# tqch/ddpm-torch

Measured on AMD Instinct MI355X. Metric: training imgs/s/GPU + 1000-step DDPM samples/s, CIFAR-10 UNet @1/2/4/8 MI355X, higher is better.
Workload: dtype bf16; 1 GPU; configs/cifar10.json UNet (35.7M params), full Trainer.step, B=128 per GPU, 32x32, T=1000, dropout 0.1, Adam+clip+EMA; global_batch=128, rccl_ranks=1, parallelism=dp1

## Files before the change

ddpm-torch_amd/csrc/attention.hip:

```cpp
#include "common.h"
#include <string.h>

namespace {

constexpr int RB = 128;
constexpr int NT = 512;

struct Opnd {
    __amdgpu_buffer_rsrc_t rsrc;
    long long ld;
};

__device__ __forceinline__ Opnd make_opnd(const bf16_t* base, long long ld, int L, int C) {
    Opnd o;
    const UniformAddr u = uniform_addr(base);
    o.rsrc = buffer_rsrc_at(u, (unsigned)(((long long)(L - 1) * ld + C) * 2));
    o.ld = ld;
    return o;
}
__device__ __forceinline__ u32x4 ldv(const Opnd& o, unsigned off) {
    return __builtin_bit_cast(u32x4, __builtin_amdgcn_raw_buffer_load_b128(o.rsrc, off, 0, 0));
}
__device__ __forceinline__ bf16x8 as_frag(const u32x4& v) { return __builtin_bit_cast(bf16x8, v); }

struct AttnArgs {
    const bf16_t *q, *k, *v;  long long qkv_ld;
    const bf16_t *o, *d_o;    long long o_ld, do_ld;
    bf16_t *out;              long long out_ld;
    bf16_t *dq, *dk, *dv;     long long dqkv_ld;
    float *lse, *dvec;
    int B, L, C, Lpad;
    float scale;
};

__device__ __forceinline__ int tile_addr(int row, int col, int pitch_b, int km) {
    return row * pitch_b + ((((col >> 3) ^ (row & km))) << 4) + (col & 7) * 2;
}

template <int NJ>
struct P1 {
    f32x16 acc[2][NJ];
    __device__ __forceinline__ void zero() {
#pragma unroll
        for (int i = 0; i < 2; ++i)
#pragma unroll
            for (int j = 0; j < NJ; ++j) acc[i][j] = (f32x16)(0.f);
    }
};

__device__ __forceinline__ void wait_vm_rt(int n) {
    switch (n) {
    case 0: asm volatile("s_waitcnt vmcnt(0)" ::: "memory"); break;
    case 1: asm volatile("s_waitcnt vmcnt(1)" ::: "memory"); break;
    case 2: asm volatile("s_waitcnt vmcnt(2)" ::: "memory"); break;
    case 3: asm volatile("s_waitcnt vmcnt(3)" ::: "memory"); break;
    case 4: asm volatile("s_waitcnt vmcnt(4)" ::: "memory"); break;
    case 5: asm volatile("s_waitcnt vmcnt(5)" ::: "memory"); break;
    case 6: asm volatile("s_waitcnt vmcnt(6)" ::: "memory"); break;
    case 7: asm volatile("s_waitcnt vmcnt(7)" ::: "memory"); break;
    default: asm volatile("s_waitcnt vmcnt(8)" ::: "memory"); break;
    }
}

#ifdef ATTN_TIMING
__device__ unsigned long long* g_attn_timing = nullptr;
#define ATTN_STAMP(slot) do { if (g_attn_timing && threadIdx.x == 0) g_attn_timing[(blockIdx.y * gridDim.x + blockIdx.x) * 8 + (slot)] = wall_clock64(); } while (0)
#else
#define ATTN_STAMP(slot)
#endif

constexpr int P1_RING = 3, P2_RING = 5;
constexpr int P2_SLOT = 2 * NT * 16;
__device__ __host__ __forceinline__ int p1_slot_bytes(int Lpad) { return RB * 128 + ((Lpad + 63) / 64) * 8192; }
__device__ __host__ __forceinline__ int p2_rows(int C) { return C > 256 ? 16 : (C > 128 ? 32 : 64); }

template <int NJ, bool PIPE = true>
__device__ __forceinline__ void product_nt(P1<NJ>& t, const Opnd& X, int r0, const Opnd& Y, int Lpad, int C, char* lds, int tid) {
    const int lane = tid & 63, wr = (tid >> 8) & 1, wc = (tid >> 6) & 3;
    const int wave = __builtin_amdgcn_readfirstlane(tid >> 6);
    const int nyi = (Lpad + 63) / 64;
    const int xs_bytes = RB * 128, slot_bytes = p1_slot_bytes(Lpad), per = 2 + nyi;
    const unsigned lds0 = lds_addr(lds);
    const int nchunks = (C + 63) / 64;
    unsigned xo[2], yo[4]; int xc[2], yc[4];
#pragma unroll
    for (int i = 0; i < 2; ++i) {
        const int v = tid + NT * i, row = v >> 3;
        xc[i] = ((v & 7) ^ ((row >> 1) & 7)) * 8;
        xo[i] = (unsigned)(((long long)(r0 + row) * X.ld + xc[i]) * 2);
    }
#pragma unroll
    for (int i = 0; i < 4; ++i) {
        const int v = tid + NT * i, row = v >> 3;
        yc[i] = ((v & 7) ^ ((row >> 1) & 7)) * 8;
        yo[i] = row < Lpad ? (unsigned)(((long long)row * Y.ld + yc[i]) * 2) : BUF_OOB;
    }
    auto issue = [&](int ch) {
        char* slot = lds + (ch % P1_RING) * slot_bytes;
        const int c0 = ch * 64;
#pragma unroll
        for (int i = 0; i < 2; ++i) {
            unsigned o = c0 + xc[i] < C ? xo[i] + (unsigned)(c0 * 2) : BUF_OOB;
            asm volatile("" : "+v"(o));
            LDS_DMA16(X.rsrc, slot + (i * NT + wave * 64) * 16, o, 0);
        }
#pragma unroll
        for (int i = 0; i < 4; ++i) {
            if (i < nyi) {
                unsigned o = (yo[i] != BUF_OOB && c0 + yc[i] < C) ? yo[i] + (unsigned)(c0 * 2) : BUF_OOB;
                asm volatile("" : "+v"(o));
                LDS_DMA16(Y.rsrc, slot + xs_bytes + (i * NT + wave * 64) * 16, o, 0);
            }
        }
    };
    issue(0);
    if (nchunks > 1) issue(1);
    const int sw = (lane >> 5) ^ ((lane >> 1) & 7);
    const unsigned arow = (unsigned)((wr * 64 + (lane & 31)) * 128), brow = (unsigned)(xs_bytes + (wc * 32 + (lane & 31)) * 128);
    bool jok[NJ];
#pragma unroll
    for (int j = 0; j < NJ; ++j) jok[j] = (wc + 4 * j) * 32 < Lpad;
#ifdef ATTN_TIMING
    unsigned long long tq[5] = {0, 0, 0, 0, 0};
#define P1_T(k) do { if (ch == 1) tq[k] = clock64(); } while (0)
#else
#define P1_T(k)
#endif
    for (int ch = 0; ch < nchunks; ++ch) {
        P1_T(0);
        wait_vm_rt(ch + 1 < nchunks ? per : 0);
        P1_T(1);
        __builtin_amdgcn_s_barrier();
        P1_T(2);
        if (ch + 2 < nchunks) issue(ch + 2);
        P1_T(3);
        const unsigned cur = lds0 + (unsigned)((ch % P1_RING) * slot_bytes);
        constexpr int NS = PIPE ? 2 : 1;
        u32x4 fa[NS][2], fb[NS][NJ];
        auto rd = [&](int kc, int set) {
            const unsigned ko = (unsigned)(((2 * kc) ^ sw) << 4);
#pragma unroll
            for (int i = 0; i < 2; ++i) fa[set][i] = lds_rd16(cur + arow + (unsigned)(i * 32 * 128) + ko);
#pragma unroll
            for (int j = 0; j < NJ; ++j) fb[set][j] = lds_rd16(cur + (jok[j] ? brow + (unsigned)(j * 128 * 128) : (unsigned)xs_bytes) + ko);
        };
        rd(0, 0);
#pragma unroll
        for (int kc = 0; kc < 4; ++kc) {
            constexpr int cs = NS == 2 ? 1 : 0;
            if (NS == 1) { if (kc > 0) rd(kc, 0); lds_wait_n<0>(); }
            else if (kc < 3) { rd(kc + 1, (kc + 1) & 1); lds_wait_n<2 + NJ>(); } else lds_wait_n<0>();
#pragma unroll
            for (int i = 0; i < 2; ++i)
#pragma unroll
                for (int j = 0; j < NJ; ++j)
                    if (jok[j]) t.acc[i][j] = __builtin_amdgcn_mfma_f32_32x32x16_bf16(as_frag(fa[kc & cs][i]), as_frag(fb[kc & cs][j]), t.acc[i][j], 0, 0, 0);
            __builtin_amdgcn_sched_barrier(0);
        }
        P1_T(4);
    }
#ifdef ATTN_TIMING
    if (g_attn_timing && threadIdx.x == 0 && tq[4])
        g_attn_timing[(blockIdx.y * gridDim.x + blockIdx.x) * 8 + 7] = ((tq[1] - tq[0]) & 0xffff) | (((tq[2] - tq[1]) & 0xffff) << 16) | (((tq[3] - tq[2]) & 0xffff) << 32) | (((tq[4] - tq[3]) & 0xffff) << 48);
#endif
#undef P1_T
    __syncthreads();
}

template <int NJ2>
__device__ __forceinline__ void product_nn(f32x16 (&z)[2][NJ2], const char* tile, int pitch_b, int km, const Opnd& Y, int L, int Lpad, int C,
                                           char* ring, int tid) {
    const int lane = tid & 63, wr = (tid >> 8) & 1, wc = (tid >> 6) & 3;
    const int wave = __builtin_amdgcn_readfirstlane(tid >> 6);
    const int KR = p2_rows(C);
    const int row_b = C * 2, cpr = C >> 3;
    const int nvec = KR * cpr;
    const int skey = C % 128 == 0 ? 2 : 0;
#pragma unroll
    for (int i = 0; i < 2; ++i)
#pragma unroll
        for (int j = 0; j < NJ2; ++j) z[i][j] = (f32x16)(0.f);
    const int nchunks = (Lpad + KR - 1) / KR;
    int vkr[2]; unsigned vo[2];
#pragma unroll
    for (int i = 0; i < 2; ++i) {
        const int v = tid + NT * i;
        const int kr = v / cpr, pc = v - kr * cpr;
        const int lc = skey ? (pc ^ ((kr & 3) << 2)) : pc;
        vkr[i] = v < nvec ? kr : (1 << 20);
        vo[i] = (unsigned)(((long long)kr * Y.ld + lc * 8) * 2);
    }
    const unsigned kstep = (unsigned)((long long)KR * Y.ld * 2);
    auto issue = [&](int ch) {
        char* slot = ring + (ch % P2_RING) * P2_SLOT;
#pragma unroll
        for (int i = 0; i < 2; ++i) {
            unsigned o = ch * KR + vkr[i] < L ? vo[i] + (unsigned)ch * kstep : BUF_OOB;
            asm volatile("" : "+v"(o));
            LDS_DMA16(Y.rsrc, slot + (i * NT + wave * 64) * 16, o, 0);
        }
    };
    for (int c = 0; c < P2_RING - 1 && c < nchunks; ++c) issue(c);
    const int i16 = lane & 15;
    const unsigned tile0 = lds_addr(tile), ring0 = lds_addr(ring);
    bool jok[NJ2];
#pragma unroll
    for (int j = 0; j < NJ2; ++j) jok[j] = (wc + 4 * j) * 32 < C;
    for (int ch = 0; ch < nchunks; ++ch) {
        const int ahead = min(ch + P2_RING - 2, nchunks - 1) - ch;
        wait_vm_rt(2 * ahead);
        __builtin_amdgcn_s_barrier();
        if (ch + P2_RING - 1 < nchunks) issue(ch + P2_RING - 1);
        const unsigned cur = ring0 + (unsigned)((ch % P2_RING) * P2_SLOT);
        constexpr int NS = NJ2 <= 2 ? 2 : 1;
        u32x4 fa[NS][2]; uint2 fb[NS][NJ2][2];
        const int nks = min(KR / 16, (Lpad - ch * KR + 15) / 16);
        auto rd = [&](int ks, int set) {
            const int kg = ch * KR + ks * 16;
#pragma unroll
            for (int i = 0; i < 2; ++i) {
                const int row = wr * 64 + i * 32 + (lane & 31);
                fa[set][i] = lds_rd16(tile0 + (unsigned)(row * pitch_b + ((((kg >> 3) + (lane >> 5)) ^ (row & km)) << 4)));
            }
#pragma unroll
            for (int j = 0; j < NJ2; ++j) {
                const int ct = jok[j] ? wc + 4 * j : wc;
                const int mcol = ct * 32 + ((lane >> 4) & 1) * 16 + (i16 & 3) * 4;
                const int krow = ks * 16 + (lane >> 5) * 8 + (i16 >> 2);
                const int pch = skey ? ((mcol >> 3) ^ ((krow & 3) << 2)) : (mcol >> 3);
                const unsigned p = cur + (unsigned)(krow * row_b + pch * 16 + (mcol & 7) * 2);
                fb[set][j][0] = lds_rd_tr(p); fb[set][j][1] = lds_rd_tr(p + (unsigned)(4 * row_b));
            }
        };
        rd(0, 0);
        for (int ks = 0; ks < nks; ks += 2) {
#pragma unroll
            for (int h = 0; h < 2; ++h) {
                if (ks + h >= nks) break;
                constexpr int cs = NS == 2 ? 1 : 0;
                const int cur_set = h & cs;
                if (NS == 1) { if (ks + h > 0) rd(ks + h, 0); lds_wait_n<0>(); }
                else if (ks + h + 1 < nks) { rd(ks + h + 1, (h + 1) & 1); lds_wait_n<2 + 2 * NJ2>(); } else lds_wait_n<0>();
#pragma unroll
                for (int j = 0; j < NJ2; ++j) {
                    if (!jok[j]) continue;
                    u32x4 b4; b4.x = fb[cur_set][j][0].x; b4.y = fb[cur_set][j][0].y; b4.z = fb[cur_set][j][1].x; b4.w = fb[cur_set][j][1].y;
#pragma unroll
                    for (int i = 0; i < 2; ++i) z[i][j] = __builtin_amdgcn_mfma_f32_32x32x16_bf16(as_frag(fa[cur_set][i]), as_frag(b4), z[i][j], 0, 0, 0);
                }
                __builtin_amdgcn_sched_barrier(0);
            }
        }
    }
    __syncthreads();
}

template <int CNT, int OFF, typename Op>
__device__ __forceinline__ float half_reduce(const float (&v)[CNT], int lane, Op&& op) {
    if constexpr (CNT == 1) return v[0];
    else {
        const bool bit = (lane & OFF) != 0;
        float o[CNT / 2];
#pragma unroll
        for (int k = 0; k < CNT / 2; ++k) {
            const float send = bit ? v[k] : v[k + CNT / 2], keep = bit ? v[k + CNT / 2] : v[k];
            o[k] = op(keep, __shfl_xor(send, OFF, 64));
        }
        return half_reduce<CNT / 2, OFF / 2>(o, lane, op);
    }
}

__device__ __forceinline__ int acc_row(int r, int lane) { return (r & 3) + 8 * (r >> 2) + 4 * (lane >> 5); }

template <int NJ, typename F>
__device__ __forceinline__ void write_tile(const P1<NJ>& t, char* tile, int pitch_b, int km, int Lpad, int tid, F&& f) {
    const int lane = tid & 63, wave = tid >> 6, wr = wave >> 2, wc = wave & 3;
#pragma unroll
    for (int i = 0; i < 2; ++i)
#pragma unroll
        for (int j = 0; j < NJ; ++j) {
            const int ct = wc + 4 * j;
            if (ct * 32 >= Lpad) continue;
#pragma unroll
            for (int r = 0; r < 16; ++r) {
                const int row = wr * 64 + i * 32 + acc_row(r, lane), col = ct * 32 + (lane & 31);
                *reinterpret_cast<bf16_t*>(tile + tile_addr(row, col, pitch_b, km)) = f2bf(f(t.acc[i][j][r], i, j, r, row, col));
            }
        }
}

template <int NJ2>
__device__ __forceinline__ void store_rows(const f32x16 (&z)[2][NJ2], bf16_t* out, long long ld, int r0, int L, int C, int tid) {
    const int lane = tid & 63, wave = tid >> 6, wr = wave >> 2, wc = wave & 3;
#pragma unroll
    for (int i = 0; i < 2; ++i)
#pragma unroll
        for (int j = 0; j < NJ2; ++j) {
            const int ct = wc + 4 * j;
            if (ct * 32 >= C) continue;
#pragma unroll
            for (int r = 0; r < 16; ++r) {
                const int row = r0 + wr * 64 + i * 32 + acc_row(r, lane);
                if (row < L) out[(long long)row * ld + ct * 32 + (lane & 31)] = f2bf(z[i][j][r]);
            }
        }
}

__device__ __forceinline__ void attn_block(int B, int& b, int& r0) {
    const int gx = gridDim.x;
    if (gx > 1 && (B & 7) == 0) {
        const int L = blockIdx.y * gx + blockIdx.x, k = L >> 3;
        r0 = (k % gx) * RB;
        b = (k / gx) * 8 + (L & 7);
    } else { b = blockIdx.y; r0 = blockIdx.x * RB; }
}

struct Lds {
    char* tile; char* stage; float* red;
    int pitch_b, km;
};
__device__ __forceinline__ Lds carve(char* smem, int Lpad) {
    Lds l;
    l.pitch_b = Lpad * 2;
    const int nch = Lpad >> 3;
    int span = 4;
    while (span < 16 && nch % (span * 2) == 0) span *= 2;
    l.km = span - 1;
    l.tile = smem;
    l.stage = smem + RB * l.pitch_b;
    l.red = nullptr;
    return l;
}

template <int NJ1, int NJ2>
__global__ __launch_bounds__(NT, 2)
void attn_fwd_lse_kernel(AttnArgs a) {
    extern __shared__ __attribute__((aligned(16))) char smem[];
    const int tid = threadIdx.x, lane = tid & 63, wave = tid >> 6, wr = wave >> 2, wc = wave & 3;
    int b, r0;
    attn_block(a.B, b, r0);
    Lds l = carve(smem, a.Lpad);
    const Opnd Q = make_opnd(a.q + (long long)b * a.L * a.qkv_ld, a.qkv_ld, a.L, a.C);
    const Opnd K = make_opnd(a.k + (long long)b * a.L * a.qkv_ld, a.qkv_ld, a.L, a.C);
    const Opnd V = make_opnd(a.v + (long long)b * a.L * a.qkv_ld, a.qkv_ld, a.L, a.C);
    ATTN_STAMP(0);
    P1<NJ1> s;
    s.zero();
    product_nt<NJ1, (NJ2 <= 2)>(s, Q, r0, K, a.Lpad, a.C, smem, tid);
    ATTN_STAMP(1);
    float* red = reinterpret_cast<float*>(l.stage);
    const int kk = lane & 31, myrow = wr * 64 + (kk >> 4) * 32 + acc_row(kk & 15, lane);
    float vals[32];
#pragma unroll
    for (int i = 0; i < 2; ++i)
#pragma unroll
        for (int r = 0; r < 16; ++r) {
            float m = -3.0e38f;
#pragma unroll
            for (int j = 0; j < NJ1; ++j) {
                const int col = (wc + 4 * j) * 32 + (lane & 31);
                const float v = col < a.L ? s.acc[i][j][r] * a.scale : -3.0e38f;
                s.acc[i][j][r] = v;
                m = fmaxf(m, v);
            }
            vals[i * 16 + r] = m;
        }
    red[wc * RB + myrow] = half_reduce<32, 16>(vals, lane, [](float x, float y) { return fmaxf(x, y); });
    __syncthreads();
#pragma unroll
    for (int i = 0; i < 2; ++i)
#pragma unroll
        for (int r = 0; r < 16; ++r) {
            const int row = wr * 64 + i * 32 + acc_row(r, lane);
            const float m = fmaxf(fmaxf(red[row], red[RB + row]), fmaxf(red[2 * RB + row], red[3 * RB + row]));
            float sum = 0.f;
#pragma unroll
            for (int j = 0; j < NJ1; ++j) {
                const int col = (wc + 4 * j) * 32 + (lane & 31);
                const float e = col < a.L ? __expf(s.acc[i][j][r] - m) : 0.f;
                s.acc[i][j][r] = e;
                sum += e;
            }
            vals[i * 16 + r] = sum;
        }
    float* rsum = red + 4 * RB;
    rsum[wc * RB + myrow] = half_reduce<32, 16>(vals, lane, [](float x, float y) { return x + y; });
    __syncthreads();
    float rinv[2][16];
#pragma unroll
    for (int i = 0; i < 2; ++i)
#pragma unroll
        for (int r = 0; r < 16; ++r) {
            const int row = wr * 64 + i * 32 + acc_row(r, lane);
            const float tot = (rsum[row] + rsum[RB + row]) + (rsum[2 * RB + row] + rsum[3 * RB + row]);
            rinv[i][r] = __builtin_amdgcn_rcpf(tot);
        }
    if (a.lse && tid < RB && r0 + tid < a.L) {
        const float m = fmaxf(fmaxf(red[tid], red[RB + tid]), fmaxf(red[2 * RB + tid], red[3 * RB + tid]));
        const float tot = (rsum[tid] + rsum[RB + tid]) + (rsum[2 * RB + tid] + rsum[3 * RB + tid]);
        a.lse[(long long)b * a.L + r0 + tid] = m + __logf(tot);
    }
    __syncthreads();
    ATTN_STAMP(2);
    write_tile<NJ1>(s, l.tile, l.pitch_b, l.km, a.Lpad, tid, [&](float e, int i, int, int r, int, int) { return e * rinv[i][r]; });
    __syncthreads();
    ATTN_STAMP(3);
    f32x16 z[2][NJ2];
    product_nn<NJ2>(z, l.tile, l.pitch_b, l.km, V, a.L, a.Lpad, a.C, l.stage, tid);
    ATTN_STAMP(4);
    store_rows<NJ2>(z, a.out + (long long)b * a.L * a.out_ld, a.out_ld, r0, a.L, a.C, tid);
    ATTN_STAMP(5);
#ifdef ATTN_TIMING
    asm volatile("s_waitcnt vmcnt(0)" ::: "memory");
#endif
    ATTN_STAMP(6);
}

template <int NJ1, int NJ2>
__global__ __launch_bounds__(NT, 2)
void attn_bwd_dq_kernel(AttnArgs a) {
    extern __shared__ __attribute__((aligned(16))) char smem[];
    const int tid = threadIdx.x, lane = tid & 63, wave = tid >> 6, wr = wave >> 2, wc = wave & 3;
    int b, r0;
    attn_block(a.B, b, r0);
    Lds l = carve(smem, a.Lpad);
    const Opnd Q = make_opnd(a.q + (long long)b * a.L * a.qkv_ld, a.qkv_ld, a.L, a.C);
    const Opnd K = make_opnd(a.k + (long long)b * a.L * a.qkv_ld, a.qkv_ld, a.L, a.C);
    const Opnd V = make_opnd(a.v + (long long)b * a.L * a.qkv_ld, a.qkv_ld, a.L, a.C);
    const Opnd dO = make_opnd(a.d_o + (long long)b * a.L * a.do_ld, a.do_ld, a.L, a.C);
    float* dloc = reinterpret_cast<float*>(l.tile);
    {
        const int row = tid >> 2, part = tid & 3, q = r0 + row;
        float acc = 0.f;
        if (q < a.L) {
            const bf16_t* po = a.o + ((long long)b * a.L + q) * a.o_ld;
            const bf16_t* pd = a.d_o + ((long long)b * a.L + q) * a.do_ld;
            for (int c = part * 8; c < a.C; c += 32) {
                float fo[8], fd[8];
                Elem<bf16_t>::unpack(ldg16(po + c), fo); Elem<bf16_t>::unpack(ldg16(pd + c), fd);
#pragma unroll
                for (int e = 0; e < 8; ++e) acc += fo[e] * fd[e];
            }
        }
        acc += __shfl_xor(acc, 1, 64); acc += __shfl_xor(acc, 2, 64);
        if (part == 0) { dloc[row] = acc; if (q < a.L) a.dvec[(long long)b * a.L + q] = acc; }
    }
    __syncthreads();
    float drow[2][16], lrow[2][16];
#pragma unroll
    for (int i = 0; i < 2; ++i)
#pragma unroll
        for (int r = 0; r < 16; ++r) {
            const int row = wr * 64 + i * 32 + acc_row(r, lane), q = r0 + row;
            drow[i][r] = dloc[row];
            lrow[i][r] = q < a.L ? a.lse[(long long)b * a.L + q] : 0.f;
        }
    __syncthreads();
    P1<NJ1> p;
    p.zero();
    product_nt<NJ1, (NJ2 <= 2)>(p, Q, r0, K, a.Lpad, a.C, smem, tid);
#pragma unroll
    for (int i = 0; i < 2; ++i)
#pragma unroll
        for (int j = 0; j < NJ1; ++j)
#pragma unroll
            for (int r = 0; r < 16; ++r) {
                const int col = (wc + 4 * j) * 32 + (lane & 31);
                p.acc[i][j][r] = col < a.L ? __expf(p.acc[i][j][r] * a.scale - lrow[i][r]) : 0.f;
            }
    P1<NJ1> dp;
    dp.zero();
    product_nt<NJ1, (NJ2 <= 2)>(dp, dO, r0, V, a.Lpad, a.C, smem, tid);
    write_tile<NJ1>(dp, l.tile, l.pitch_b, l.km, a.Lpad, tid,
                    [&](float v, int i, int j, int r, int, int) { return p.acc[i][j][r] * (v - drow[i][r]) * a.scale; });
    __syncthreads();
    f32x16 z[2][NJ2];
    product_nn<NJ2>(z, l.tile, l.pitch_b, l.km, K, a.L, a.Lpad, a.C, l.stage, tid);
    store_rows<NJ2>(z, a.dq + (long long)b * a.L * a.dqkv_ld, a.dqkv_ld, r0, a.L, a.C, tid);
}

template <int NJ1, int NJ2>
__global__ __launch_bounds__(NT, 2)
void attn_bwd_dkv_kernel(AttnArgs a) {
    extern __shared__ __attribute__((aligned(16))) char smem[];
    const int tid = threadIdx.x, lane = tid & 63, wave = tid >> 6, wc = wave & 3;
    int b, r0;
    attn_block(a.B, b, r0);
    Lds l = carve(smem, a.Lpad);
    const Opnd Q = make_opnd(a.q + (long long)b * a.L * a.qkv_ld, a.qkv_ld, a.L, a.C);
    const Opnd K = make_opnd(a.k + (long long)b * a.L * a.qkv_ld, a.qkv_ld, a.L, a.C);
    const Opnd V = make_opnd(a.v + (long long)b * a.L * a.qkv_ld, a.qkv_ld, a.L, a.C);
    const Opnd dO = make_opnd(a.d_o + (long long)b * a.L * a.do_ld, a.do_ld, a.L, a.C);
    float lcol[NJ1], dcol[NJ1];
#pragma unroll
    for (int j = 0; j < NJ1; ++j) {
        const int q = (wc + 4 * j) * 32 + (lane & 31);
        lcol[j] = q < a.L ? a.lse[(long long)b * a.L + q] : 0.f;
        dcol[j] = q < a.L ? a.dvec[(long long)b * a.L + q] : 0.f;
    }
    P1<NJ1> p;
    p.zero();
    product_nt<NJ1, (NJ2 <= 2)>(p, K, r0, Q, a.Lpad, a.C, smem, tid);
#pragma unroll
    for (int i = 0; i < 2; ++i)
#pragma unroll
        for (int j = 0; j < NJ1; ++j)
#pragma unroll
            for (int r = 0; r < 16; ++r) {
                const int q = (wc + 4 * j) * 32 + (lane & 31);
                p.acc[i][j][r] = q < a.L ? __expf(p.acc[i][j][r] * a.scale - lcol[j]) : 0.f;
            }
    write_tile<NJ1>(p, l.tile, l.pitch_b, l.km, a.Lpad, tid, [&](float v, int, int, int, int, int) { return v; });
    __syncthreads();
    f32x16 z[2][NJ2];
    product_nn<NJ2>(z, l.tile, l.pitch_b, l.km, dO, a.L, a.Lpad, a.C, l.stage, tid);
    store_rows<NJ2>(z, a.dv + (long long)b * a.L * a.dqkv_ld, a.dqkv_ld, r0, a.L, a.C, tid);
    P1<NJ1> dp;
    dp.zero();
    product_nt<NJ1, (NJ2 <= 2)>(dp, V, r0, dO, a.Lpad, a.C, smem, tid);
    write_tile<NJ1>(dp, l.tile, l.pitch_b, l.km, a.Lpad, tid,
                    [&](float v, int i, int j, int r, int, int) { return p.acc[i][j][r] * (v - dcol[j]) * a.scale; });
    __syncthreads();
    product_nn<NJ2>(z, l.tile, l.pitch_b, l.km, Q, a.L, a.Lpad, a.C, l.stage, tid);
    store_rows<NJ2>(z, a.dk + (long long)b * a.L * a.dqkv_ld, a.dqkv_ld, r0, a.L, a.C, tid);
}

static int check_common(const void* qkv, long long ld, int B, int L, int C, int dtype) {
    if (!qkv) return DDPM_ERR_NULL;
    if (dtype != DDPM_BF16) return DDPM_ERR_DTYPE;
    if (B <= 0 || L <= 0 || L > 256 || L % 16 || C <= 0 || C > 512 || C % 32 || ld < 3 * C) return DDPM_ERR_SHAPE;
    if (!aligned16(qkv) || ld % 8) return DDPM_ERR_ALIGN;
    if ((long long)L * ld * 2 > BUF_OOB) return DDPM_ERR_SHAPE;
    return DDPM_OK;
}

static size_t lds_bytes(int Lpad, int C) {
    const size_t tile = (size_t)RB * Lpad * 2;
    const int nch1 = (C + 63) / 64, nch2 = (Lpad + p2_rows(C) - 1) / p2_rows(C);
    const size_t p1 = (size_t)(nch1 < P1_RING ? nch1 : P1_RING) * p1_slot_bytes(Lpad);
    size_t p2 = (size_t)(nch2 < P2_RING ? nch2 : P2_RING) * P2_SLOT;
    const size_t red = 8 * RB * sizeof(float);
    if (p2 < red) p2 = red;
    return p1 > tile + p2 ? p1 : tile + p2;
}

#define ATTN_DISPATCH(KERNEL, grid, lds, st, a)                                                                            \
    do {                                                                                                                   \
        const int nj1 = (a.Lpad / 32 + 3) / 4, nj2 = (a.C / 32 + 3) / 4;                                                   \
        auto go = [&](auto k) -> int {                                                                                     \
            if (hipFuncSetAttribute(reinterpret_cast<const void*>(k), hipFuncAttributeMaxDynamicSharedMemorySize, 160 * 1024) != hipSuccess) return DDPM_ERR_LAUNCH; \
            hipLaunchKernelGGL(k, grid, dim3(NT), lds, st, a);                                                             \
            return check_launch();                                                                                         \
        };                                                                                                                 \
        if (nj1 <= 1 && nj2 <= 1) return go(&KERNEL<1, 1>);                                                                \
        if (nj1 <= 1 && nj2 <= 2) return go(&KERNEL<1, 2>);                                                                \
        if (nj1 <= 1) return go(&KERNEL<1, 4>);                                                                            \
        if (nj2 <= 1) return go(&KERNEL<2, 1>);                                                                            \
        if (nj2 <= 2) return go(&KERNEL<2, 2>);                                                                            \
        return go(&KERNEL<2, 4>);                                                                                          \
    } while (0)

}

#ifdef ATTN_TIMING
extern "C" int ddpm_debug_set_attn_timing(void* p) { return hipMemcpyToSymbol(HIP_SYMBOL(g_attn_timing), &p, sizeof(p)) == hipSuccess ? 0 : -1; }
#endif

extern "C" int ddpm_attention_fwd_lse(const void* qkv, long long ld, void* out, long long out_ld, float* lse, int B, int L, int C, float scale,
                                      int dtype, void* stream) {
    int rc = check_common(qkv, ld, B, L, C, dtype);
    if (rc) return rc;
    if (!out) return DDPM_ERR_NULL;
    if (!aligned16(out) || out_ld % 8) return DDPM_ERR_ALIGN;
    AttnArgs a; memset(&a, 0, sizeof(a));
    a.q = (const bf16_t*)qkv; a.k = a.q + C; a.v = a.q + 2 * C; a.qkv_ld = ld;
    a.out = (bf16_t*)out; a.out_ld = out_ld; a.lse = lse;
    a.B = B; a.L = L; a.C = C; a.Lpad = (L + 31) / 32 * 32; a.scale = scale;
    const dim3 grid((L + RB - 1) / RB, B);
    const size_t lds = lds_bytes(a.Lpad, C);
    hipStream_t st = (hipStream_t)stream;
    ATTN_DISPATCH(attn_fwd_lse_kernel, grid, lds, st, a);
}

extern "C" int ddpm_attention_bwd(const void* qkv, long long ld, const void* o, long long o_ld, const void* d_o, long long do_ld,
                                  const float* lse, float* dvec, void* dqkv, long long dqkv_ld, int B, int L, int C, float scale,
                                  int dtype, void* stream) {
    int rc = check_common(qkv, ld, B, L, C, dtype);
    if (rc) return rc;
    if (!o || !d_o || !lse || !dvec || !dqkv) return DDPM_ERR_NULL;
    if (!aligned16(o) || !aligned16(d_o) || !aligned16(dqkv) || o_ld % 8 || do_ld % 8 || dqkv_ld % 8 || dqkv_ld < 3 * C) return DDPM_ERR_ALIGN;
    AttnArgs a; memset(&a, 0, sizeof(a));
    a.q = (const bf16_t*)qkv; a.k = a.q + C; a.v = a.q + 2 * C; a.qkv_ld = ld;
    a.o = (const bf16_t*)o; a.o_ld = o_ld; a.d_o = (const bf16_t*)d_o; a.do_ld = do_ld;
    a.dq = (bf16_t*)dqkv; a.dk = a.dq + C; a.dv = a.dq + 2 * C; a.dqkv_ld = dqkv_ld;
    a.lse = const_cast<float*>(lse); a.dvec = dvec;
    a.B = B; a.L = L; a.C = C; a.Lpad = (L + 31) / 32 * 32; a.scale = scale;
    const dim3 grid((L + RB - 1) / RB, B);
    const size_t lds = lds_bytes(a.Lpad, C);
    hipStream_t st = (hipStream_t)stream;
    {
        auto run = [&]() -> int { ATTN_DISPATCH(attn_bwd_dq_kernel, grid, lds, st, a); };
        rc = run();
        if (rc) return rc;
    }
    ATTN_DISPATCH(attn_bwd_dkv_kernel, grid, lds, st, a);
}
```

Baseline: 14490 imgs/s.

## Overlap attention stage loads with prior compute and vectorize tile writes

Restructures the attention forward and backward kernels so the next product's global-to-LDS DMA loads are issued before the current stage finishes (prefetch of V/K/Q/dO rings, primed product calls, prologue/epilogue hooks). Row vectors and dV stores are folded into product loops, and a dedicated aux LDS region replaces the reuse of the tile buffer. Accumulator tile and output writes are packed with DPP/perm into 64-bit stores instead of scalar bf16 stores. This aims to hide memory latency and cut LDS write instructions, at the cost of more LDS use and riskier synchronisation (syncthreads replaced by bare s_barrier).

New measurement: 14570 imgs/s, median of 6. About the same (+0.6%).

```diff
diff --git a/ddpm-torch_amd/csrc/attention.hip b/ddpm-torch_amd/csrc/attention.hip
--- a/ddpm-torch_amd/csrc/attention.hip
+++ b/ddpm-torch_amd/csrc/attention.hip
@@ -31,6 +31,7 @@
     float *lse, *dvec;
     int B, L, C, Lpad;
     float scale;
+    int aux_off;
 };
 
 __device__ __forceinline__ int tile_addr(int row, int col, int pitch_b, int km) {
@@ -64,57 +65,86 @@
 
 #ifdef ATTN_TIMING
 __device__ unsigned long long* g_attn_timing = nullptr;
-#define ATTN_STAMP(slot) do { if (g_attn_timing && threadIdx.x == 0) g_attn_timing[(blockIdx.y * gridDim.x + blockIdx.x) * 8 + (slot)] = wall_clock64(); } while (0)
+#define ATTN_STAMP_AT(k, slot) do { if (g_attn_timing && threadIdx.x == 0) g_attn_timing[(((k) * gridDim.y + blockIdx.y) * gridDim.x + blockIdx.x) * 8 + (slot)] = wall_clock64(); } while (0)
 #else
-#define ATTN_STAMP(slot)
+#define ATTN_STAMP_AT(k, slot)
 #endif
+#define ATTN_STAMP(slot) ATTN_STAMP_AT(0, slot)
 
 constexpr int P1_RING = 3, P2_RING = 5;
 constexpr int P2_SLOT = 2 * NT * 16;
 __device__ __host__ __forceinline__ int p1_slot_bytes(int Lpad) { return RB * 128 + ((Lpad + 63) / 64) * 8192; }
 __device__ __host__ __forceinline__ int p2_rows(int C) { return C > 256 ? 16 : (C > 128 ? 32 : 64); }
 
-template <int NJ, bool PIPE = true>
-__device__ __forceinline__ void product_nt(P1<NJ>& t, const Opnd& X, int r0, const Opnd& Y, int Lpad, int C, char* lds, int tid) {
-    const int lane = tid & 63, wr = (tid >> 8) & 1, wc = (tid >> 6) & 3;
-    const int wave = __builtin_amdgcn_readfirstlane(tid >> 6);
-    const int nyi = (Lpad + 63) / 64;
-    const int xs_bytes = RB * 128, slot_bytes = p1_slot_bytes(Lpad), per = 2 + nyi;
-    const unsigned lds0 = lds_addr(lds);
-    const int nchunks = (C + 63) / 64;
+__device__ __forceinline__ void lds_wr16(unsigned addr, unsigned v) { asm volatile("ds_write_b16 %0, %1" :: "v"(addr), "v"(v) : "memory"); }
+__device__ __forceinline__ void lds_wr32(unsigned addr, float v) { asm volatile("ds_write_b32 %0, %1" :: "v"(addr), "v"(v) : "memory"); }
+__device__ __forceinline__ void lds_wr64(unsigned addr, uint2 v) { asm volatile("ds_write_b64 %0, %1" :: "v"(addr), "v"(v) : "memory"); }
+
+
+struct P1Load {
+    __amdgpu_buffer_rsrc_t xr, yr;
     unsigned xo[2], yo[4]; int xc[2], yc[4];
-#pragma unroll
-    for (int i = 0; i < 2; ++i) {
-        const int v = tid + NT * i, row = v >> 3;
-        xc[i] = ((v & 7) ^ ((row >> 1) & 7)) * 8;
-        xo[i] = (unsigned)(((long long)(r0 + row) * X.ld + xc[i]) * 2);
-    }
-#pragma unroll
-    for (int i = 0; i < 4; ++i) {
-        const int v = tid + NT * i, row = v >> 3;
-        yc[i] = ((v & 7) ^ ((row >> 1) & 7)) * 8;
-        yo[i] = row < Lpad ? (unsigned)(((long long)row * Y.ld + yc[i]) * 2) : BUF_OOB;
-    }
-    auto issue = [&](int ch) {
-        char* slot = lds + (ch % P1_RING) * slot_bytes;
+    int nyi, C;
+    __device__ __forceinline__ P1Load(const Opnd& X, int r0, const Opnd& Y, int Lpad, int C_, int tid) : xr(X.rsrc), yr(Y.rsrc), C(C_) {
+        nyi = (Lpad + 63) / 64;
+#pragma unroll
+        for (int i = 0; i < 2; ++i) {
+            const int v = tid + NT * i, row = v >> 3;
+            xc[i] = ((v & 7) ^ ((row >> 1) & 7)) * 8;
+            xo[i] = (unsigned)(((long long)(r0 + row) * X.ld + xc[i]) * 2);
+        }
+#pragma unroll
+        for (int i = 0; i < 4; ++i) {
+            const int v = tid + NT * i, row = v >> 3;
+            yc[i] = ((v & 7) ^ ((row >> 1) & 7)) * 8;
+            yo[i] = row < Lpad ? (unsigned)(((long long)row * Y.ld + yc[i]) * 2) : BUF_OOB;
+        }
+    }
+    __device__ __forceinline__ void issue(int ch, char* slot, int wave) const {
         const int c0 = ch * 64;
 #pragma unroll
         for (int i = 0; i < 2; ++i) {
             unsigned o = c0 + xc[i] < C ? xo[i] + (unsigned)(c0 * 2) : BUF_OOB;
             asm volatile("" : "+v"(o));
-            LDS_DMA16(X.rsrc, slot + (i * NT + wave * 64) * 16, o, 0);
+            LDS_DMA16(xr, slot + (i * NT + wave * 64) * 16, o, 0);
         }
 #pragma unroll
         for (int i = 0; i < 4; ++i) {
             if (i < nyi) {
                 unsigned o = (yo[i] != BUF_OOB && c0 + yc[i] < C) ? yo[i] + (unsigned)(c0 * 2) : BUF_OOB;
                 asm volatile("" : "+v"(o));
-                LDS_DMA16(Y.rsrc, slot + xs_bytes + (i * NT + wave * 64) * 16, o, 0);
-            }
-        }
-    };
-    issue(0);
-    if (nchunks > 1) issue(1);
+                LDS_DMA16(yr, slot + RB * 128 + (i * NT + wave * 64) * 16, o, 0);
+            }
+        }
+    }
+};
+
+__device__ __forceinline__ void p1_prefetch(const Opnd& X, int r0, const Opnd& Y, int Lpad, int C, char* lds, int tid, int seq0) {
+    const int wave = __builtin_amdgcn_readfirstlane(tid >> 6);
+    const int slot_bytes = p1_slot_bytes(Lpad);
+    const P1Load ld(X, r0, Y, Lpad, C, tid);
+    ld.issue(0, lds + (seq0 % P1_RING) * slot_bytes, wave);
+    if (C > 64) ld.issue(1, lds + ((seq0 + 1) % P1_RING) * slot_bytes, wave);
+}
+
+struct NoHook { __device__ __forceinline__ void operator()() const {} };
+
+template <int NJ, bool PIPE = true, typename Pro = NoHook, typename Epi = NoHook>
+__device__ __forceinline__ void product_nt(P1<NJ>& t, const Opnd& X, int r0, const Opnd& Y, int Lpad, int C, char* lds, int tid,
+                                           int seq0 = 0, bool primed = false, bool end_sync = true, Pro&& pro = Pro(), Epi&& epi = Epi()) {
+    const int lane = tid & 63, wr = (tid >> 8) & 1, wc = (tid >> 6) & 3;
+    const int wave = __builtin_amdgcn_readfirstlane(tid >> 6);
+    const int xs_bytes = RB * 128, slot_bytes = p1_slot_bytes(Lpad);
+    const unsigned lds0 = lds_addr(lds);
+    const int nchunks = (C + 63) / 64;
+    const P1Load ld(X, r0, Y, Lpad, C, tid);
+    const int per = 2 + ld.nyi;
+    auto issue = [&](int ch) { ld.issue(ch, lds + ((seq0 + ch) % P1_RING) * slot_bytes, wave); };
+    if (!primed) {
+        issue(0);
+        if (nchunks > 1) issue(1);
+    }
+    pro();
     const int sw = (lane >> 5) ^ ((lane >> 1) & 7);
     const unsigned arow = (unsigned)((wr * 64 + (lane & 31)) * 128), brow = (unsigned)(xs_bytes + (wc * 32 + (lane & 31)) * 128);
     bool jok[NJ];
@@ -133,8 +163,9 @@
         __builtin_amdgcn_s_barrier();
         P1_T(2);
         if (ch + 2 < nchunks) issue(ch + 2);
+        if (ch + 1 == nchunks) epi();
         P1_T(3);
-        const unsigned cur = lds0 + (unsigned)((ch % P1_RING) * slot_bytes);
+        const unsigned cur = lds0 + (unsigned)(((seq0 + ch) % P1_RING) * slot_bytes);
         constexpr int NS = PIPE ? 2 : 1;
         u32x4 fa[NS][2], fb[NS][NJ];
         auto rd = [&](int kc, int set) {
@@ -164,43 +195,63 @@
         g_attn_timing[(blockIdx.y * gridDim.x + blockIdx.x) * 8 + 7] = ((tq[1] - tq[0]) & 0xffff) | (((tq[2] - tq[1]) & 0xffff) << 16) | (((tq[3] - tq[2]) & 0xffff) << 32) | (((tq[4] - tq[3]) & 0xffff) << 48);
 #endif
 #undef P1_T
-    __syncthreads();
+    if (end_sync) __syncthreads();
+}
+
+struct P2Load {
+    __amdgpu_buffer_rsrc_t yr;
+    int vkr[2]; unsigned vo[2]; unsigned kstep;
+    int KR, L;
+    __device__ __forceinline__ P2Load(const Opnd& Y, int L_, int C, int tid) : yr(Y.rsrc), L(L_) {
+        KR = p2_rows(C);
+        const int cpr = C >> 3;
+        const int nvec = KR * cpr;
+        const int skey = C % 128 == 0 ? 2 : 0;
+#pragma unroll
+        for (int i = 0; i < 2; ++i) {
+            const int v = tid + NT * i;
+            const int kr = v / cpr, pc = v - kr * cpr;
+            const int lc = skey ? (pc ^ ((kr & 3) << 2)) : pc;
+            vkr[i] = v < nvec ? kr : (1 << 20);
+            vo[i] = (unsigned)(((long long)kr * Y.ld + lc * 8) * 2);
+        }
+        kstep = (unsigned)((long long)KR * Y.ld * 2);
+    }
+    __device__ __forceinline__ void issue(int ch, char* ring, int wave) const {
+        char* slot = ring + (ch % P2_RING) * P2_SLOT;
+#pragma unroll
+        for (int i = 0; i < 2; ++i) {
+            unsigned o = ch * KR + vkr[i] < L ? vo[i] + (unsigned)ch * kstep : BUF_OOB;
+            asm volatile("" : "+v"(o));
+            LDS_DMA16(yr, slot + (i * NT + wave * 64) * 16, o, 0);
+        }
+    }
+};
+
+__device__ __forceinline__ void p2_prefetch(const Opnd& Y, int L, int Lpad, int C, char* ring, int tid) {
+    const int wave = __builtin_amdgcn_readfirstlane(tid >> 6);
+    const int KR = p2_rows(C), nchunks = (Lpad + KR - 1) / KR;
+    const P2Load ld(Y, L, C, tid);
+    for (int c = 0; c < P2_RING - 1 && c < nchunks; ++c) ld.issue(c, ring, wave);
 }
 
 template <int NJ2>
 __device__ __forceinline__ void product_nn(f32x16 (&z)[2][NJ2], const char* tile, int pitch_b, int km, const Opnd& Y, int L, int Lpad, int C,
-                                           char* ring, int tid) {
+                                           char* ring, int tid, bool primed = false) {
     const int lane = tid & 63, wr = (tid >> 8) & 1, wc = (tid >> 6) & 3;
     const int wave = __builtin_amdgcn_readfirstlane(tid >> 6);
     const int KR = p2_rows(C);
-    const int row_b = C * 2, cpr = C >> 3;
-    const int nvec = KR * cpr;
+    const int row_b = C * 2;
     const int skey = C % 128 == 0 ? 2 : 0;
 #pragma unroll
     for (int i = 0; i < 2; ++i)
 #pragma unroll
         for (int j = 0; j < NJ2; ++j) z[i][j] = (f32x16)(0.f);
     const int nchunks = (Lpad + KR - 1) / KR;
-    int vkr[2]; unsigned vo[2];
-#pragma unroll
-    for (int i = 0; i < 2; ++i) {
-        const int v = tid + NT * i;
-        const int kr = v / cpr, pc = v - kr * cpr;
-        const int lc = skey ? (pc ^ ((kr & 3) << 2)) : pc;
-        vkr[i] = v < nvec ? kr : (1 << 20);
-        vo[i] = (unsigned)(((long long)kr * Y.ld + lc * 8) * 2);
-    }
-    const unsigned kstep = (unsigned)((long long)KR * Y.ld * 2);
-    auto issue = [&](int ch) {
-        char* slot = ring + (ch % P2_RING) * P2_SLOT;
-#pragma unroll
-        for (int i = 0; i < 2; ++i) {
-            unsigned o = ch * KR + vkr[i] < L ? vo[i] + (unsigned)ch * kstep : BUF_OOB;
-            asm volatile("" : "+v"(o));
-            LDS_DMA16(Y.rsrc, slot + (i * NT + wave * 64) * 16, o, 0);
-        }
-    };
-    for (int c = 0; c < P2_RING - 1 && c < nchunks; ++c) issue(c);
+    const P2Load ld(Y, L, C, tid);
+    auto issue = [&](int ch) { ld.issue(ch, ring, wave); };
+    if (!primed)
+        for (int c = 0; c < P2_RING - 1 && c < nchunks; ++c) issue(c);
     const int i16 = lane & 15;
     const unsigned tile0 = lds_addr(tile), ring0 = lds_addr(ring);
     bool jok[NJ2];
@@ -272,9 +323,25 @@
 
 __device__ __forceinline__ int acc_row(int r, int lane) { return (r & 3) + 8 * (r >> 2) + 4 * (lane >> 5); }
 
+__device__ __forceinline__ uint2 quad_rows(float v0, float v1, float v2, float v3, int lane) {
+    const bool odd = (lane & 1) != 0, up = (lane & 2) != 0;
+    const unsigned sel = odd ? 0x03020706u : 0x05040100u;
+    const unsigned p01 = pack_bf2(v0, v1), p23 = pack_bf2(v2, v3);
+    const unsigned g01 = (unsigned)__builtin_amdgcn_mov_dpp((int)p01, 0xB1, 0xf, 0xf, true);
+    const unsigned g23 = (unsigned)__builtin_amdgcn_mov_dpp((int)p23, 0xB1, 0xf, 0xf, true);
+    const unsigned a = __builtin_amdgcn_perm(g01, p01, sel);
+    const unsigned b = __builtin_amdgcn_perm(g23, p23, sel);
+    const unsigned got = (unsigned)__builtin_amdgcn_mov_dpp((int)(up ? a : b), 0x4E, 0xf, 0xf, true);
+    uint2 o;
+    o.x = up ? got : a;
+    o.y = up ? b : got;
+    return o;
+}
+
 template <int NJ, typename F>
 __device__ __forceinline__ void write_tile(const P1<NJ>& t, char* tile, int pitch_b, int km, int Lpad, int tid, F&& f) {
     const int lane = tid & 63, wave = tid >> 6, wr = wave >> 2, wc = wave & 3;
+    const unsigned tile0 = lds_addr(tile);
 #pragma unroll
     for (int i = 0; i < 2; ++i)
 #pragma unroll
@@ -282,11 +349,14 @@
             const int ct = wc + 4 * j;
             if (ct * 32 >= Lpad) continue;
 #pragma unroll
-            for (int r = 0; r < 16; ++r) {
-                const int row = wr * 64 + i * 32 + acc_row(r, lane), col = ct * 32 + (lane & 31);
-                *reinterpret_cast<bf16_t*>(tile + tile_addr(row, col, pitch_b, km)) = f2bf(f(t.acc[i][j][r], i, j, r, row, col));
-            }
-        }
+            for (int g = 0; g < 4; ++g) {
+                const int rb = wr * 64 + i * 32 + acc_row(4 * g, lane), col = ct * 32 + (lane & 31);
+                const uint2 o = quad_rows(f(t.acc[i][j][4 * g], i, j, 4 * g, rb, col), f(t.acc[i][j][4 * g + 1], i, j, 4 * g + 1, rb + 1, col),
+                                          f(t.acc[i][j][4 * g + 2], i, j, 4 * g + 2, rb + 2, col), f(t.acc[i][j][4 * g + 3], i, j, 4 * g + 3, rb + 3, col), lane);
+                lds_wr64(tile0 + (unsigned)tile_addr(rb + (lane & 3), col & ~3, pitch_b, km), o);
+            }
+        }
+    lds_wait();
 }
 
 template <int NJ2>
@@ -298,10 +368,19 @@
         for (int j = 0; j < NJ2; ++j) {
             const int ct = wc + 4 * j;
             if (ct * 32 >= C) continue;
-#pragma unroll
-            for (int r = 0; r < 16; ++r) {
-                const int row = r0 + wr * 64 + i * 32 + acc_row(r, lane);
-                if (row < L) out[(long long)row * ld + ct * 32 + (lane & 31)] = f2bf(z[i][j][r]);
+            if constexpr (NJ2 > 2) {
+#pragma unroll
+                for (int r = 0; r < 16; ++r) {
+                    const int row = r0 + wr * 64 + i * 32 + acc_row(r, lane);
+                    if (row < L) out[(long long)row * ld + ct * 32 + (lane & 31)] = f2bf(z[i][j][r]);
+                }
+                continue;
+            }
+#pragma unroll
+            for (int g = 0; g < 4; ++g) {
+                const uint2 o = quad_rows(z[i][j][4 * g], z[i][j][4 * g + 1], z[i][j][4 * g + 2], z[i][j][4 * g + 3], lane);
+                const int row = r0 + wr * 64 + i * 32 + acc_row(4 * g, lane) + (lane & 3);
+                if (row < L) *reinterpret_cast<uint2*>(out + (long long)row * ld + ct * 32 + (lane & 28)) = o;
             }
         }
 }
@@ -337,6 +416,7 @@
 void attn_fwd_lse_kernel(AttnArgs a) {
     extern __shared__ __attribute__((aligned(16))) char smem[];
     const int tid = threadIdx.x, lane = tid & 63, wave = tid >> 6, wr = wave >> 2, wc = wave & 3;
+    constexpr bool EARLY = NJ2 <= 2;
     int b, r0;
     attn_block(a.B, b, r0);
     Lds l = carve(smem, a.Lpad);
@@ -402,11 +482,12 @@
     }
     __syncthreads();
     ATTN_STAMP(2);
+    if (EARLY) p2_prefetch(V, a.L, a.Lpad, a.C, l.stage, tid);
     write_tile<NJ1>(s, l.tile, l.pitch_b, l.km, a.Lpad, tid, [&](float e, int i, int, int r, int, int) { return e * rinv[i][r]; });
-    __syncthreads();
+    __builtin_amdgcn_s_barrier();
     ATTN_STAMP(3);
     f32x16 z[2][NJ2];
-    product_nn<NJ2>(z, l.tile, l.pitch_b, l.km, V, a.L, a.Lpad, a.C, l.stage, tid);
+    product_nn<NJ2>(z, l.tile, l.pitch_b, l.km, V, a.L, a.Lpad, a.C, l.stage, tid, EARLY);
     ATTN_STAMP(4);
     store_rows<NJ2>(z, a.out + (long long)b * a.L * a.out_ld, a.out_ld, r0, a.L, a.C, tid);
     ATTN_STAMP(5);
@@ -428,8 +509,12 @@
     const Opnd K = make_opnd(a.k + (long long)b * a.L * a.qkv_ld, a.qkv_ld, a.L, a.C);
     const Opnd V = make_opnd(a.v + (long long)b * a.L * a.qkv_ld, a.qkv_ld, a.L, a.C);
     const Opnd dO = make_opnd(a.d_o + (long long)b * a.L * a.do_ld, a.do_ld, a.L, a.C);
-    float* dloc = reinterpret_cast<float*>(l.tile);
-    {
+    ATTN_STAMP(0);
+    constexpr bool EARLY = NJ2 <= 2;
+    const int nch = (a.C + 63) / 64;
+    float* aux = reinterpret_cast<float*>(smem + a.aux_off);
+    const unsigned aux0 = lds_addr(aux);
+    auto row_vectors = [&]() {
         const int row = tid >> 2, part = tid & 3, q = r0 + row;
         float acc = 0.f;
         if (q < a.L) {
@@ -443,22 +528,23 @@
             }
         }
         acc += __shfl_xor(acc, 1, 64); acc += __shfl_xor(acc, 2, 64);
-        if (part == 0) { dloc[row] = acc; if (q < a.L) a.dvec[(long long)b * a.L + q] = acc; }
-    }
-    __syncthreads();
-    float drow[2][16], lrow[2][16];
-#pragma unroll
-    for (int i = 0; i < 2; ++i)
-#pragma unroll
-        for (int r = 0; r < 16; ++r) {
-            const int row = wr * 64 + i * 32 + acc_row(r, lane), q = r0 + row;
-            drow[i][r] = dloc[row];
-            lrow[i][r] = q < a.L ? a.lse[(long long)b * a.L + q] : 0.f;
-        }
-    __syncthreads();
+        if (part == 0) { lds_wr32(aux0 + (unsigned)(row * 4), acc); if (q < a.L) a.dvec[(long long)b * a.L + q] = acc; }
+        if (tid < RB) lds_wr32(aux0 + (unsigned)((RB + tid) * 4), r0 + tid < a.L ? a.lse[(long long)b * a.L + r0 + tid] : 0.f);
+        lds_wait();
+        ATTN_STAMP(1);
+    };
+    float lrow[2][16];
+    auto s_tail = [&]() {
+#pragma unroll
+        for (int i = 0; i < 2; ++i)
+#pragma unroll
+            for (int r = 0; r < 16; ++r) lrow[i][r] = aux[RB + wr * 64 + i * 32 + acc_row(r, lane)];
+        if (EARLY) p1_prefetch(dO, r0, V, a.Lpad, a.C, smem, tid, nch);
+    };
     P1<NJ1> p;
     p.zero();
-    product_nt<NJ1, (NJ2 <= 2)>(p, Q, r0, K, a.Lpad, a.C, smem, tid);
+    product_nt<NJ1, (NJ2 <= 2)>(p, Q, r0, K, a.Lpad, a.C, smem, tid, 0, false, !EARLY, row_vectors, s_tail);
+    ATTN_STAMP(2);
 #pragma unroll
     for (int i = 0; i < 2; ++i)
 #pragma unroll
@@ -470,13 +556,23 @@
             }
     P1<NJ1> dp;
     dp.zero();
-    product_nt<NJ1, (NJ2 <= 2)>(dp, dO, r0, V, a.Lpad, a.C, smem, tid);
+    product_nt<NJ1, (NJ2 <= 2)>(dp, dO, r0, V, a.Lpad, a.C, smem, tid, nch, EARLY);
+    ATTN_STAMP(3);
+    float drow[2][16];
+#pragma unroll
+    for (int i = 0; i < 2; ++i)
+#pragma unroll
+        for (int r = 0; r < 16; ++r) drow[i][r] = aux[wr * 64 + i * 32 + acc_row(r, lane)];
+    if (EARLY) p2_prefetch(K, a.L, a.Lpad, a.C, l.stage, tid);
     write_tile<NJ1>(dp, l.tile, l.pitch_b, l.km, a.Lpad, tid,
                     [&](float v, int i, int j, int r, int, int) { return p.acc[i][j][r] * (v - drow[i][r]) * a.scale; });
-    __syncthreads();
+    __builtin_amdgcn_s_barrier();
+    ATTN_STAMP(4);
     f32x16 z[2][NJ2];
-    product_nn<NJ2>(z, l.tile, l.pitch_b, l.km, K, a.L, a.Lpad, a.C, l.stage, tid);
+    product_nn<NJ2>(z, l.tile, l.pitch_b, l.km, K, a.L, a.Lpad, a.C, l.stage, tid, EARLY);
+    ATTN_STAMP(5);
     store_rows<NJ2>(z, a.dq + (long long)b * a.L * a.dqkv_ld, a.dqkv_ld, r0, a.L, a.C, tid);
+    ATTN_STAMP(6);
 }
 
 template <int NJ1, int NJ2>
@@ -491,16 +587,23 @@
     const Opnd K = make_opnd(a.k + (long long)b * a.L * a.qkv_ld, a.qkv_ld, a.L, a.C);
     const Opnd V = make_opnd(a.v + (long long)b * a.L * a.qkv_ld, a.qkv_ld, a.L, a.C);
     const Opnd dO = make_opnd(a.d_o + (long long)b * a.L * a.do_ld, a.do_ld, a.L, a.C);
+    ATTN_STAMP_AT(1, 0);
+    constexpr bool EARLY = NJ2 <= 2;
+    const int nch = (a.C + 63) / 64;
     float lcol[NJ1], dcol[NJ1];
-#pragma unroll
-    for (int j = 0; j < NJ1; ++j) {
-        const int q = (wc + 4 * j) * 32 + (lane & 31);
-        lcol[j] = q < a.L ? a.lse[(long long)b * a.L + q] : 0.f;
-        dcol[j] = q < a.L ? a.dvec[(long long)b * a.L + q] : 0.f;
-    }
+    auto col_vectors = [&]() {
+#pragma unroll
+        for (int j = 0; j < NJ1; ++j) {
+            const int q = (wc + 4 * j) * 32 + (lane & 31);
+            lcol[j] = q < a.L ? a.lse[(long long)b * a.L + q] : 0.f;
+            dcol[j] = q < a.L ? a.dvec[(long long)b * a.L + q] : 0.f;
+        }
+    };
     P1<NJ1> p;
     p.zero();
-    product_nt<NJ1, (NJ2 <= 2)>(p, K, r0, Q, a.Lpad, a.C, smem, tid);
+    product_nt<NJ1, (NJ2 <= 2)>(p, K, r0, Q, a.Lpad, a.C, smem, tid, 0, false, true, col_vectors);
+    ATTN_STAMP_AT(1, 1);
+    if (EARLY) p2_prefetch(dO, a.L, a.Lpad, a.C, l.stage, tid);
 #pragma unroll
     for (int i = 0; i < 2; ++i)
 #pragma unroll
@@ -511,18 +614,24 @@
                 p.acc[i][j][r] = q < a.L ? __expf(p.acc[i][j][r] * a.scale - lcol[j]) : 0.f;
             }
     write_tile<NJ1>(p, l.tile, l.pitch_b, l.km, a.Lpad, tid, [&](float v, int, int, int, int, int) { return v; });
-    __syncthreads();
+    __builtin_amdgcn_s_barrier();
+    ATTN_STAMP_AT(1, 2);
     f32x16 z[2][NJ2];
-    product_nn<NJ2>(z, l.tile, l.pitch_b, l.km, dO, a.L, a.Lpad, a.C, l.stage, tid);
-    store_rows<NJ2>(z, a.dv + (long long)b * a.L * a.dqkv_ld, a.dqkv_ld, r0, a.L, a.C, tid);
+    product_nn<NJ2>(z, l.tile, l.pitch_b, l.km, dO, a.L, a.Lpad, a.C, l.stage, tid, EARLY);
+    ATTN_STAMP_AT(1, 3);
+    auto store_dv = [&]() { store_rows<NJ2>(z, a.dv + (long long)b * a.L * a.dqkv_ld, a.dqkv_ld, r0, a.L, a.C, tid); };
     P1<NJ1> dp;
     dp.zero();
-    product_nt<NJ1, (NJ2 <= 2)>(dp, V, r0, dO, a.Lpad, a.C, smem, tid);
+    product_nt<NJ1, (NJ2 <= 2)>(dp, V, r0, dO, a.Lpad, a.C, smem, tid, nch, false, true, store_dv);
+    ATTN_STAMP_AT(1, 4);
+    if (EARLY) p2_prefetch(Q, a.L, a.Lpad, a.C, l.stage, tid);
     write_tile<NJ1>(dp, l.tile, l.pitch_b, l.km, a.Lpad, tid,
                     [&](float v, int i, int j, int r, int, int) { return p.acc[i][j][r] * (v - dcol[j]) * a.scale; });
-    __syncthreads();
-    product_nn<NJ2>(z, l.tile, l.pitch_b, l.km, Q, a.L, a.Lpad, a.C, l.stage, tid);
+    __builtin_amdgcn_s_barrier();
+    product_nn<NJ2>(z, l.tile, l.pitch_b, l.km, Q, a.L, a.Lpad, a.C, l.stage, tid, EARLY);
+    ATTN_STAMP_AT(1, 5);
     store_rows<NJ2>(z, a.dk + (long long)b * a.L * a.dqkv_ld, a.dqkv_ld, r0, a.L, a.C, tid);
+    ATTN_STAMP_AT(1, 6);
 }
 
 static int check_common(const void* qkv, long long ld, int B, int L, int C, int dtype) {
@@ -536,13 +645,14 @@
 
 static size_t lds_bytes(int Lpad, int C) {
     const size_t tile = (size_t)RB * Lpad * 2;
-    const int nch1 = (C + 63) / 64, nch2 = (Lpad + p2_rows(C) - 1) / p2_rows(C);
-    const size_t p1 = (size_t)(nch1 < P1_RING ? nch1 : P1_RING) * p1_slot_bytes(Lpad);
+    const int nch2 = (Lpad + p2_rows(C) - 1) / p2_rows(C);
+    const size_t p1 = (size_t)P1_RING * p1_slot_bytes(Lpad);
     size_t p2 = (size_t)(nch2 < P2_RING ? nch2 : P2_RING) * P2_SLOT;
     const size_t red = 8 * RB * sizeof(float);
     if (p2 < red) p2 = red;
     return p1 > tile + p2 ? p1 : tile + p2;
 }
+constexpr size_t AUX_BYTES = 2 * RB * sizeof(float);
 
 #define ATTN_DISPATCH(KERNEL, grid, lds, st, a)                                                                            \
     do {                                                                                                                   \
@@ -577,7 +687,8 @@
     a.out = (bf16_t*)out; a.out_ld = out_ld; a.lse = lse;
     a.B = B; a.L = L; a.C = C; a.Lpad = (L + 31) / 32 * 32; a.scale = scale;
     const dim3 grid((L + RB - 1) / RB, B);
-    const size_t lds = lds_bytes(a.Lpad, C);
+    a.aux_off = (int)lds_bytes(a.Lpad, C);
+    const size_t lds = (size_t)a.aux_off + AUX_BYTES;
     hipStream_t st = (hipStream_t)stream;
     ATTN_DISPATCH(attn_fwd_lse_kernel, grid, lds, st, a);
 }
@@ -596,7 +707,8 @@
     a.lse = const_cast<float*>(lse); a.dvec = dvec;
     a.B = B; a.L = L; a.C = C; a.Lpad = (L + 31) / 32 * 32; a.scale = scale;
     const dim3 grid((L + RB - 1) / RB, B);
-    const size_t lds = lds_bytes(a.Lpad, C);
+    a.aux_off = (int)lds_bytes(a.Lpad, C);
+    const size_t lds = (size_t)a.aux_off + AUX_BYTES;
     hipStream_t st = (hipStream_t)stream;
     {
         auto run = [&]() -> int { ATTN_DISPATCH(attn_bwd_dq_kernel, grid, lds, st, a); };
```
